# adolliou/euispice_coreg

Hardware: AMD Instinct MI355X
Metric: lag-points/sec (whole node) on 2048² grid, 60×60 CRVAL sweep; argmax-shift match (higher is better)
Workload: dtype f64; 1 GPU; headline: Carrington 'fa' 2048x2048 grid lon(200,300) lat(-20,20), 60x60 CRVAL lags arange(-30,30,1) arcsec, small 2048^2 HRIEUV-like, ref 3072^2 FSI-like, order 2, solar_r 1.004; lag_points=3600, parallelism=single GPU, no collective, resident=True, sweeps_in_flight=2, small_stored_f32=True, use_lds=True

## Files before the change

euispice_coreg_amd/_lib.py:

```python
from __future__ import annotations

import ctypes as C
import os

import numpy as np

_HERE = os.path.dirname(os.path.abspath(__file__))
LIB_PATH = os.environ.get("COREG_HIP_LIB", os.path.join(_HERE, "libcoreg_hip.so"))

COREG_OK = 0
COREG_EINVAL, COREG_EHIP, COREG_ESTATE, COREG_ENOTIMPL, COREG_ENOMEM = -1, -2, -3, -4, -5
COREG_F32, COREG_F64 = 0, 1
PROJ_TAN, PROJ_CAR = 0, 1
METHOD_CORRELATION, METHOD_RESIDUS, METHOD_RESIDUS_MASKED = 0, 1, 2
METHOD_MUTUAL_INFORMATION = 3
CDELT_INTENDED, CDELT_REFERENCE = 0, 1


class CoregError(RuntimeError):
    def __init__(self, code, msg):
        super().__init__(f"libcoreg_hip error {code}: {msg}")
        self.code = code


# ... 211 lines not shown
     [_P, _WP, C.POINTER(CarrGrid), C.c_double, C.POINTER(Lags), C.c_int, C.c_int, C.c_int, C.c_int64, C.c_int64, _P,
      C.c_int]),
    ("coreg_sweep_set_bins", C.c_int, [_P, _P, C.c_int32, _P, C.c_int32]),
    ("coreg_sweep_helioprojective", C.c_int,
     [_P, _WP, _WP, C.POINTER(Lags), C.c_int, C.c_int, C.c_int, C.c_int64, C.c_int64, _P, C.c_int]),
    ("coreg_sums_size", C.c_int, [_P, C.POINTER(C.c_int64)]),
    ("coreg_copy_sums", C.c_int, [_P, _P, C.c_int]),
    ("coreg_finalize_sums", C.c_int, [_P, _P, C.c_int, _P, C.c_int]),
    ("coreg_get_pivots", C.c_int, [_P, C.POINTER(C.c_double)]),
    ("coreg_set_pivots", C.c_int, [_P, C.POINTER(C.c_double)]),
    ("coreg_last_stats", C.c_int, [_P, C.POINTER(Stats)]),
    ("coreg_last_counts", C.c_int, [_P, _P, C.c_int]),
    ("coreg_last_visit_counts", C.c_int, [_P, C.POINTER(C.c_int64)]),
    ("coreg_last_tap_fix", C.c_int, [_P, C.POINTER(C.c_int64)]),
    ("coreg_last_sweep_variant", C.c_int, [_P, C.POINTER(C.c_int32)]),
    ("coreg_set_option", C.c_int, [_P, C.c_char_p, C.c_int64]),
    ("coreg_shift_header", C.c_int,
     [_WP, C.c_double, C.c_double, C.c_double, C.c_double, C.c_double, C.c_int, _WP]),
    ("coreg_homography", C.c_int, [_WP, _WP, C.POINTER(C.c_double)]),
    ("coreg_lag_homography", C.c_int,
     [_WP, _WP, C.POINTER(Lags), C.POINTER(C.c_int32), C.c_int, C.POINTER(C.c_double)]),
    ("coreg_carrington_origin", C.c_int, [_WP, C.POINTER(C.c_double), C.POINTER(C.c_double)]),
    ("coreg_diffrot_table", C.c_int, [C.POINTER(CarrGrid), C.POINTER(DiffRot), _P]),
    ("coreg_car_map", C.c_int, [_WP, _WP, C.c_int64, _P, _P, _P, _P]),
    ("coreg_wcslib_pixel_to_pixel", C.c_int, [_WP, _WP, C.c_int64, _P, _P, _P, _P, _P, _P]),
    ("coreg_car_tile_margin", C.c_int, [_WP, _WP, C.c_int32, C.c_double, C.POINTER(C.c_double)]),
    ("coreg_nansum_planes_be", C.c_int, [_P, C.c_int32, C.c_int64, _P, C.c_int32, _P]),
    ("coreg_fit_gaussian2d", C.c_int,
     [C.c_int32, _P, _P, _P, _P, _P, _P, C.c_int32, C.c_double, C.c_double, C.c_double, C.c_int32, _P,
      C.POINTER(C.c_int32), C.POINTER(C.c_int32)]),
# ... 558 lines not shown
        self._chk(self._lib.coreg_finalize_sums(self._h, _P(sptr), s_dev, _P(int(out_dev_ptr)), 1))
        return None

    def get_pivots(self):
        p = (C.c_double * 2)()
        self._chk(self._lib.coreg_get_pivots(self._h, p))
        return float(p[0]), float(p[1])

    def set_pivots(self, pivot_ref, pivot_small):
        p = (C.c_double * 2)(float(pivot_ref), float(pivot_small))
        self._chk(self._lib.coreg_set_pivots(self._h, p))

    def last_stats(self) -> dict:
        s = Stats()
        self._chk(self._lib.coreg_last_stats(self._h, C.byref(s)))
        return {f: getattr(s, f) for f, _ in Stats._fields_}

    def last_counts(self, dst_ptr=None):
        n = getattr(self, "_counts_n", None)
        if n is None:
            raise CoregError(COREG_ESTATE, "last_counts: no sweep has run through this object")
        if dst_ptr is not None:
            self._chk(self._lib.coreg_last_counts(self._h, _P(int(dst_ptr)), 1))
            return None
        out = np.empty(int(n), dtype=np.float64)
        self._chk(self._lib.coreg_last_counts(self._h, out.ctypes.data, 0))
        return out

    def last_visit_counts(self) -> dict:
        c = (C.c_int64 * 6)()
        self._chk(self._lib.coreg_last_visit_counts(self._h, c))
# ... 360 lines not shown
```

euispice_coreg_amd/csrc/abi_host.hpp:

```cpp
#pragma once
extern "C" {
int coreg_shift_header(const coreg_wcs2d* ref, double d_crval1, double d_crval2, double d_cdelt1, double d_cdelt2,
                       double d_crota, int cdelt_semantics, coreg_wcs2d* out) {
    if (!ref || !out) return COREG_EINVAL;
    return shift_header(*ref, d_crval1, d_crval2, d_cdelt1, d_cdelt2, d_crota, cdelt_semantics, out);
}

int coreg_car_map(const coreg_wcs2d* from, const coreg_wcs2d* to, int64_t n, const double* px, const double* py,
                  double* ox, double* oy) {
    if (!from || !to || n < 0 || (n > 0 && (!px || !py || !ox || !oy))) return COREG_EINVAL;
    if (from->proj != COREG_PROJ_CAR || to->proj != COREG_PROJ_CAR) return COREG_EINVAL;
    CarMapHost m;
    if (m.init(*from, *to)) return 1;
    for (int64_t i = 0; i < n; ++i) m.apply(px[i], py[i], &ox[i], &oy[i]);
    return COREG_OK;
}

int coreg_last_visit_counts(coreg_handle* h, int64_t* counts6) {
    int64_t* counts5 = counts6;
    if (!h || !counts5) return COREG_EINVAL;
    RETCHK(bind_device(h));
    HIPCHK(hipStreamSynchronize(h->stream));
    long long info[8] = {0, 0, 0, 0, 0, 0, 0, 0};
    if (h->tile_info.p) HIPCHK(hipMemcpy(info, h->tile_info.p, 7 * sizeof(long long), hipMemcpyDeviceToHost));
// ... 2 lines not shown
    if (h->counters.p) HIPCHK(hipMemcpy(refined, h->counters.p, sizeof(refined), hipMemcpyDeviceToHost));
    counts5[4] = refined[0];
    counts6[5] = refined[1];
    return COREG_OK;
}

int coreg_last_tap_fix(coreg_handle* h, int64_t* counts3) {
    if (!h || !counts3) return COREG_EINVAL;
    for (int k = 0; k < 3; ++k) counts3[k] = h->tap_last[k];
    return COREG_OK;
}

int coreg_last_sweep_variant(coreg_handle* h, int32_t* v7) {
    if (!h || !v7) return COREG_EINVAL;
    for (int k = 0; k < 7; ++k) v7[k] = h->last_variant[k];
    return COREG_OK;
}

int coreg_car_tile_margin(const coreg_wcs2d* hdr_target, const coreg_wcs2d* hdr_shifted, int32_t tile_w,
                          double tile_abs_lat_rad, double* margin_px) {
    if (!hdr_target || !hdr_shifted || !margin_px || tile_w < 1 || tile_w > kTilePts) return COREG_EINVAL;
    if (hdr_target->proj != COREG_PROJ_CAR || hdr_shifted->proj != COREG_PROJ_CAR) return COREG_EINVAL;
    CarMapHost m;
    if (m.init(*hdr_target, *hdr_shifted)) return 1;
    *margin_px = car_tile_margin(car_box_c(*hdr_target, *hdr_shifted, tile_w), tile_abs_lat_rad + car_pole_sep(m.r));
    return COREG_OK;
}

int coreg_homography(const coreg_wcs2d* from, const coreg_wcs2d* to, double* h9) {
    if (!from || !to || !h9) return COREG_EINVAL;
// ... 118 lines not shown
```

euispice_coreg_amd/csrc/abi_images.hpp:

```cpp
#pragma once
extern "C" {
static int check_image(coreg_handle* h, const void* img, int32_t ny, int32_t nx, const char* who) {
    if (!img || ny < 1 || nx < 1 || too_many(ny, nx))
        return fail(h, COREG_EINVAL, std::string(who) + ": bad image (null pointer, empty, or more than 2^31 - 1 pixels)");
    return COREG_OK;
}
static bool is_dtype(int dtype) { return dtype == COREG_F32 || dtype == COREG_F64; }

static int adopt_small(coreg_handle* h, int32_t ny, int32_t nx, bool f32, hipStream_t s) {
    h->sW = nx;
    h->sH = ny;
    h->small_f32 = f32;
    HIPCHK(buffer_mean(h, h->small.p, f32, (long long)ny * nx, h->pivots.as<double>() + 1, s));
    return end_small_upload(h, s);
}

static int set_small_from(coreg_handle* h, const void* src, const PixFmt& fmt, SrcKind kind, int32_t ny, int32_t nx) {
    RETCHK(check_image(h, src, ny, nx, "set_small"));
    const size_t n = (size_t)ny * nx;
    if (kind == SRC_HOST && (fmt.raw() ? fmt.swap_only() : fmt.f32)) {
        trace("set_small_f32: enter");
        RETCHK(bind_device(h));
        HIPCHK(h->small.reserve(n * sizeof(float)));
        hipStream_t s;
        RETCHK(begin_small_upload(h, &s));
        if (h->opt_async_upload && s != h->stream) {
            h->small_f32 = true;
            h->sW = nx;
            h->sH = ny;
            void* dev = h->small.p;
            const bool swap32 = fmt.raw();
            post_upload(h, [h, dev, src, n, swap32, s] { return upload_small_worker(h, dev, src, n, swap32, s); });
            h->small_pending = true;
            trace("set_small_f32: handed to the upload thread");
            return COREG_OK;
        }
        RETCHK(staged_upload(h, h->small.p, src, n * sizeof(float), s));
        if (fmt.raw()) fits_swap32(h->small.p, n, s);
        RETCHK(adopt_small(h, ny, nx, true, s));
        trace("set_small_f32: issued");
        return COREG_OK;
    }
    RETCHK(bind_device(h));
    bool f32 = true;
// ... 110 lines not shown
        const int64_t len = coregrice::rice_encode_tile(q.data(), npx, blocksize, bytepix, heap + used, heap_cap - used);
        if (len < 0) return COREG_ENOMEM;
        tile_offset[n] = used;
        tile_nbytes[n] = (int32_t)len;
        used += len;
    }
    *heap_used = used;
    return COREG_OK;
}

int coreg_threshold_small(coreg_handle* h, int has_min, double vmin, int has_max, double vmax, long long* n_finite) {
    if (!h) return COREG_EINVAL;
    if (!h->small.p) return fail(h, COREG_ESTATE, "coreg_set_small has not been called");
    RETCHK(bind_device(h));
    const long long n = (long long)h->sW * h->sH;
    if (has_min || has_max) {
        const int nb = (int)std::min<long long>((n + 255) / 256, 2048);
        if (h->small_f32)
            hipLaunchKernelGGL((k_threshold<float>), dim3(nb), dim3(256), 0, h->stream, h->small.as<float>(), n, has_min,
                               vmin, has_max, vmax);
        else
            hipLaunchKernelGGL((k_threshold<double>), dim3(nb), dim3(256), 0, h->stream, h->small.as<double>(), n, has_min,
                               vmin, has_max, vmax);
        HIPCHK(hipGetLastError());
    }
    HIPCHK(buffer_mean(h, h->small.p, h->small_f32, n, h->pivots.as<double>() + 1, h->stream));
    if (n_finite) {
        long long cnt[256];
        HIPCHK(hipMemcpyAsync(cnt, h->red_cnt.p, sizeof(cnt), hipMemcpyDeviceToHost, h->stream));
        HIPCHK(hipStreamSynchronize(h->stream));
// ... 356 lines not shown
```

euispice_coreg_amd/csrc/abi_sweeps.hpp:

```cpp
#pragma once
namespace {

int check_method(coreg_handle* h, int method, bool mi_ok) {
    if (method == COREG_METHOD_MUTUAL_INFORMATION) {
        if (!mi_ok)
            return fail(h, COREG_ENOTIMPL, "method COREG_METHOD_MUTUAL_INFORMATION is a score of coreg_sweep_carrington only: the "
                                           "noise-decided samples of the other header-shift sweeps are corrected as Pearson sums");
        return check_sweep_mi(h);
    }
    if (method != COREG_METHOD_CORRELATION && method != COREG_METHOD_RESIDUS && method != COREG_METHOD_RESIDUS_MASKED)
        return fail(h, COREG_ENOTIMPL,
                    "method must be COREG_METHOD_CORRELATION, COREG_METHOD_RESIDUS or COREG_METHOD_RESIDUS_MASKED");
    return COREG_OK;
}

template <typename OwnChecks>
int open_sweep(coreg_handle* h, ComboRange combo, OwnChecks own_checks, const coreg_lags* lags, int order, int method,
               bool mi_ok, int sem, int64_t lag_begin, int64_t lag_end, int grid_w, int grid_h, const char* grid_what,
               double* corr_out, int out_on_device, SweepCall* call) {
    RETCHK(check_method(h, method, mi_ok));
    RETCHK(check_order(h, order));
    RETCHK(own_checks());
    RETCHK(check_lags(h, lags, &call->d, lag_begin, lag_end, combo));
    RETCHK(bind_device_nowait(h));
// ... 261 lines not shown
}

int coreg_get_pivots(coreg_handle* h, double* pivots2) {
    if (!h || !pivots2) return COREG_EINVAL;
    RETCHK(bind_device(h));
    HIPCHK(hipMemcpyAsync(pivots2, h->pivots.p, 2 * sizeof(double), hipMemcpyDeviceToHost, h->stream));
    HIPCHK(hipStreamSynchronize(h->stream));
    return COREG_OK;
}

int coreg_set_pivots(coreg_handle* h, const double* pivots2) {
    if (!h || !pivots2) return COREG_EINVAL;
    if (!(pivots2[0] == pivots2[0]) || !(pivots2[1] == pivots2[1]) || std::isinf(pivots2[0]) || std::isinf(pivots2[1]))
        return fail(h, COREG_EINVAL, "set_pivots: pivots must be finite");
    RETCHK(bind_device(h));
    HIPCHK(hipMemcpyAsync(h->pivots.p, pivots2, 2 * sizeof(double), hipMemcpyHostToDevice, h->stream));
    HIPCHK(hipStreamSynchronize(h->stream));
    return COREG_OK;
}

int coreg_last_counts(coreg_handle* h, double* dst, int dst_on_device) {
    if (!h) return COREG_EINVAL;
    if (h->counts_n < 0) return fail(h, COREG_ESTATE, "last_counts: no sweep has run on this handle");
    if (!dst && h->counts_n > 0) return fail(h, COREG_EINVAL, "last_counts: dst is null");
    RETCHK(bind_device(h));
    if (h->counts_n > 0)
        HIPCHK(hipMemcpyAsync(dst, h->counts.p, (size_t)h->counts_n * sizeof(double),
                              dst_on_device ? hipMemcpyDeviceToDevice : hipMemcpyDeviceToHost, h->stream));
    HIPCHK(hipStreamSynchronize(h->stream));
    return COREG_OK;
// ... 12 lines not shown
```

euispice_coreg_amd/csrc/coreg_hip.hip:

```cpp
#include <hip/hip_runtime.h>

#include <algorithm>
#include <chrono>
#include <cmath>
#include <cstdio>
#include <cstdlib>
#include <cstring>
#include <limits>
#include <condition_variable>
#include <map>
#include <memory>
#include <mutex>
#include <string>
#include <thread>
#include <functional>
#include <type_traits>
#include <utility>
#include <vector>

#include "fit.hpp"
#include "geometry.hpp"
#include "kernels.hpp"
#include <atomic>
#include "ricecomp.hpp"
// ... 82 lines not shown

int coreg_synchronize(coreg_handle* h) {
    if (!h) return COREG_EINVAL;
    RETCHK(bind_device(h));
    HIPCHK(hipStreamSynchronize(h->stream));
    return COREG_OK;
}

int coreg_set_option(coreg_handle* h, const char* name, int64_t value) {
    if (!h || !name) return COREG_EINVAL;
    const std::string n(name);
    if (n == "use_lds") {
        h->opt_use_lds = value ? 1 : 0;
    } else if (n == "clean_path") {
        h->opt_clean_path = value ? 1 : 0;
    } else if (n == "tap_nan_filter") {
        if (value < 0 || value > 2) return fail(h, COREG_EINVAL, "tap_nan_filter must be 0, 1 or 2");
        h->opt_tap_nan_filter = value;
    } else if (n == "overlap_upload") {
        h->opt_overlap_upload = value ? 1 : 0;
    } else if (n == "async_upload") {
        h->opt_async_upload = value ? 1 : 0;
    } else if (n == "refine") {
        h->opt_refine = value ? 1 : 0;
    } else if (n == "refine_cond_log10") {
        if (value < -3 || value > 15) return fail(h, COREG_EINVAL, "refine_cond_log10 must be in [-3, 15]");
        h->opt_refine_cond_log10 = value;
    } else if (n == "refine_max") {
        if (value < 0 || value > 16) return fail(h, COREG_EINVAL, "refine_max must be in [0, 16]");
    } else if (n == "tile_w") {
// ... 76 lines not shown
```

euispice_coreg_amd/csrc/host_state.hpp:

```cpp
#pragma once
namespace {

enum SrcKind {
    SRC_HOST = 0,
    SRC_PINNED = 1,
    SRC_DEVICE = 2,
    SRC_TILED = 3,
};

struct PixFmt {
    int bitpix = 0;
    bool f32 = false;
    double bscale = 1.0, bzero = 0.0;
    bool raw() const { return bitpix != 0; }
    bool scaled() const { return bscale != 1.0 || bzero != 0.0; }
    size_t elem() const { return raw() ? (size_t)(bitpix < 0 ? -bitpix : bitpix) / 8 : (f32 ? 4 : 8); }
    bool swap_only() const { return bitpix == -32 && !scaled(); }
    static PixFmt native(bool is_f32) {
        PixFmt f;
        f.f32 = is_f32;
        return f;
    }
};

// ... 29 lines not shown
struct ContextState;
struct PixelsState;

struct coreg_handle {
    int device = 0;
    Stream stream;
    std::string err;

    std::unique_ptr<ContextState> ctx;
    std::unique_ptr<PixelsState> pix;
    ~coreg_handle();

    DevBuf small;
    int sW = 0, sH = 0;
    bool small_f32 = false;
    DevBuf ref;
    int gW = 0, gH = 0;
    int ref_dtype = -1;
    DevBuf pivots, red_sum, red_cnt;
    DevBuf t_sin_lon, t_cos_lon, t_cos_lat, t_sin_lat, t_lon_deg, t_dx;
    coreg_diffrot rot_ref = {}, rot_small = {};
    bool has_rot_ref = false, has_rot_small = false;
    CarrTables tabs;
    std::vector<double> tabs_key;
    bool tabs_uploaded = false;
    PinBuf pin_img[2];
    Event ev_img[2];
    int pin_img_next = 0;
    DevBuf pts, tile_count, tile_list, tile_cum, group_first, tile_info, tile_bbox;
    DevBuf visit_rec;
// ... 67 lines not shown
    int64_t opt_crop_reference = 1;
    int64_t opt_taper_min = 128, opt_taper_frac = -1, opt_taper_rounds = 6;
    int64_t opt_use_lds = 1, opt_clean_path = 1, opt_refine = 1, opt_refine_cond_log10 = 5, opt_tile_w = 0, opt_n_groups = 0, opt_lds_bytes = (159 * 1024 * kPointGroups) / 4, opt_patch_w = 0, opt_h_series = 1, opt_h_incr = 1, opt_tile_skip = 1, opt_pitch = -1;

    coreg_stats stats;
    bool stats_pending = false;
    PinBuf pin_info;
    std::vector<EventPair> ev_sweep, ev_pre;
    size_t ev_sweep_used = 0, ev_pre_used = 0;
    hipEvent_t ev_t1 = nullptr;
    Event ev_end[2];
    PinBuf pin_plan[2];
    int plan_slot = 0;
    bool plan_open = false;
};
```

euispice_coreg_amd/csrc/host_sweep_io.hpp:

```cpp
#pragma once
namespace {
int collect_stats(coreg_handle* h);

void reset_stats(coreg_handle* h, long long n_grid_points, long long n_lags) {
    std::memset(&h->stats, 0, sizeof(h->stats));
    h->stats.small_is_f32 = h->small_f32 ? 1 : 0;
    h->stats.n_grid_points = n_grid_points;
    h->stats.n_lags = n_lags;
}

int begin_sweep(coreg_handle* h, long long n_out, double* corr_out, int out_on_device, double** out_dev) {
    h->stats_pending = false;
    h->pending_fin.clear();
    h->sums_slots = 0;
    h->pending_n_out = 0;
    h->tap_last[0] = h->tap_last[1] = h->tap_last[2] = 0;
    h->last_variant[0] = -1;
    std::memset(&h->pending_prologue, 0, sizeof(h->pending_prologue));
    if (h->plan_open) {
        h->plan_open = false;
        RETCHK(bind_device(h));
        HIPCHK(hipStreamSynchronize(h->stream));
    }
    if (!h->small.p) return fail(h, COREG_ESTATE, "coreg_set_small has not been called");
    if (!h->ref.p) return fail(h, COREG_ESTATE, "no reference image on the target grid");
    if (!corr_out && n_out > 0) return fail(h, COREG_EINVAL, "corr_out is null");
    h->ev_sweep_used = 0;
    h->ev_pre_used = 0;
    reset_stats(h, (long long)h->gW * h->gH, n_out);
    if (out_on_device) {
        *out_dev = corr_out;
    } else {
// ... 108 lines not shown
```

euispice_coreg_amd/csrc/host_sweep_launch.hpp:

```cpp
#pragma once
namespace {
using sweep_variant::SweepVariant;
static_assert(sweep_variant::kTranslate == MODE_TRANSLATE && sweep_variant::kHomography == MODE_HOMOGRAPHY &&
                  sweep_variant::kHomographySeries == MODE_HOMOGRAPHY_SERIES && sweep_variant::kCar == MODE_CAR &&
                  sweep_variant::kOrderRt == ORDER_RT, "sweep_variant.hpp restates the kernels' constants");

struct SweepLaunchSpec {
    int mode = MODE_TRANSLATE;
    int order = 2;
    int method = COREG_METHOD_CORRELATION;
    size_t slot_off = 0;
    int n_batches = 0, n_tiles = 0;
    long long lag_begin = 0;
    double* out_dev = nullptr;
    const LaunchU* car_inv = nullptr;
    const BorderFix* fix = nullptr;
    int pitch_sel = 0;
    long long n_slots() const { return (long long)n_batches * kBlock; }
    bool residus() const { return method != COREG_METHOD_CORRELATION; }
    int residus_kind() const { return method == COREG_METHOD_RESIDUS_MASKED ? 2 : (residus() ? 1 : 0); }
    const double* params_dev(const coreg_handle* h) const {
        return h->lane_params.as<double>() + (mode == MODE_TRANSLATE ? 2 : 9) * slot_off;
    }
    const long long* outidx_dev(const coreg_handle* h) const { return h->out_index.as<long long>() + slot_off; }
};

struct SweepKernel {
    void (*fn)(const SweepArgs);
    size_t attr_bytes[kMaxDevices];
};
template <size_t... I>
SweepKernel* sweep_kernel_table(std::index_sequence<I...>) {
    constexpr const SweepVariant* v = sweep_variant::kSweepVariants.v;
    static SweepKernel table[] = {
        {k_sweep<v[I].mode, v[I].order, std::conditional_t<v[I].f32, float, double>, v[I].round, v[I].resid, v[I].pitch>, {0}}...};
    return table;
}

int raise_dynamic_lds(coreg_handle* h, SweepKernel* k, size_t lds_bytes) {
    std::lock_guard<std::mutex> lock(g_attr_mutex);
    size_t& ab = k->attr_bytes[h->device % kMaxDevices];
    if (lds_bytes > 48 * 1024 && lds_bytes > ab) {
        HIPCHK(hipFuncSetAttribute((const void*)k->fn, hipFuncAttributeMaxDynamicSharedMemorySize, (int)lds_bytes));
        ab = lds_bytes;
    }
    return COREG_OK;
}

int sweep_grid(coreg_handle* h, const SweepKernel* k, size_t lds_bytes, long long items, unsigned* grid) {
    long long resident = h->opt_sweep_wgs;
// ... 1 lines not shown
        if (h->n_cus <= 0) HIPCHK(hipDeviceGetAttribute(&h->n_cus, hipDeviceAttributeMultiprocessorCount, h->device));
        int per_cu = 0;
        for (const coreg_handle::SweepResidency& r : h->sweep_residency)
            if (r.fn == (const void*)k->fn && r.lds_bytes == lds_bytes) per_cu = r.per_cu;
        if (per_cu <= 0) {
            HIPCHK(hipOccupancyMaxActiveBlocksPerMultiprocessor(&per_cu, (const void*)k->fn, kSweepThreads, lds_bytes));
            if (per_cu <= 0) return fail(h, COREG_EHIP, "launch_sweep: the device holds no k_sweep workgroup of this LDS size");
            h->sweep_residency.push_back({(const void*)k->fn, lds_bytes, per_cu});
        }
        resident = (long long)h->n_cus * per_cu;
    }
    *grid = (unsigned)(8 * ((std::min(items, resident) + 7) / 8));
    return COREG_OK;
}

int launch_k_sweep(coreg_handle* h, const SweepLaunchSpec& L, SweepArgs a, int n_groups8, size_t lds_bytes) {
    const SweepVariant v = sweep_variant::pick_sweep_variant(L.mode, L.order, h->small_f32, L.residus(), L.pitch_sel);
    const int at = sweep_variant::sweep_variant_index(v);
    if (at < 0) return fail(h, COREG_EINVAL, "launch_sweep: no k_sweep instantiation for this mode / order / pitch");
    SweepKernel* k = sweep_kernel_table(std::make_index_sequence<sweep_variant::kNumSweepVariants>()) + at;
    EventPair* ev = next_event(h, h->ev_sweep, h->ev_sweep_used);
    if (!ev) return fail(h, COREG_EHIP, "hipEventCreate failed");
    RETCHK(raise_dynamic_lds(h, k, lds_bytes));
    a.items8 = n_groups8 * L.n_batches;
    unsigned grid = 0;
    RETCHK(sweep_grid(h, k, lds_bytes, 8LL * a.items8, &grid));
    HIPCHK(h->sweep_queue.reserve(8 * sizeof(unsigned)));
    a.queue = h->sweep_queue.as<unsigned>();
    HIPCHK(hipMemsetAsync(a.queue, 0, 8 * sizeof(unsigned), h->stream));
    HIPCHK(hipEventRecord(ev->a, h->stream));
    hipLaunchKernelGGL(k->fn, dim3(grid), dim3(kSweepThreads), lds_bytes, h->stream, a);
    HIPCHK(hipEventRecord(ev->b, h->stream));
    HIPCHK(hipGetLastError());
    const int rec[7] = {at, v.mode, v.order, v.f32 ? 1 : 0, v.round ? 1 : 0, v.resid ? 1 : 0, v.pitch};
    std::copy(rec, rec + 7, h->last_variant);
// ... 13 lines not shown
    a.tile_info = h->tile_info.as<long long>();
    a.tile_bbox = h->tile_bbox.as<double>();
    a.visit_rec = h->visit_rec.as<VisitRec>();
    a.lane_params = L.params_dev(h);
    a.n_slots = L.n_slots();
    a.n_batches = L.n_batches;
    a.n_groups = n_groups;
    a.group_lo = group_lo;
    a.partials = h->partials.as<double>();
    a.queue = nullptr;
    a.items8 = 0;
    a.pivots = h->pivots.as<double>();
    a.use_lds = h->opt_use_lds ? 1 : 0;
    a.clean_path = h->opt_clean_path ? 1 : 0;
    a.lds_elems = (int)(lds_bytes / sizeof(double));
    a.car_inv = L.car_inv ? *L.car_inv : LaunchU{};
    a.car_inv.order_rt = L.order;
    a.car_inv.h_incr = (int)h->opt_h_incr;
    return a;
}

template <typename Args>
void fill_fix_common(Args& x, const coreg_handle* h, const SweepLaunchSpec& L) {
    x.img = h->small.p;
    x.W = h->sW;
    x.H = h->sH;
    x.ref = h->ref.p;
    x.ref_f32 = h->ref_dtype == COREG_F32 ? 1 : 0;
    x.gw = h->gW;
    x.order = L.order;
    x.round_f32 = L.mode == MODE_TRANSLATE ? 0 : 1;
    x.residus = L.residus() ? 1 : 0;
    x.pivots = h->pivots.as<double>();
    x.hom = L.params_dev(h);
// ... 70 lines not shown
    return COREG_OK;
}

int launch_sweep(coreg_handle* h, const SweepLaunchSpec& L) {
    const long long n_slots = L.n_slots();
    const int n_groups = pick_groups(h, L.n_batches, L.n_tiles);
    const bool sharded = h->opt_shard_world > 1;
    const int g_per = sharded ? n_groups / (int)h->opt_shard_world : n_groups;
    const int g_lo = sharded ? g_per * (int)h->opt_shard_rank : 0;
    const bool fixing = L.fix && L.fix->any() && (!sharded || h->opt_shard_rank == 0);
    HIPCHK(h->partials.reserve((size_t)(g_per + (fixing ? 1 : 0)) * kNumSums * n_slots * sizeof(double)));
    double* fix_slab = fixing ? h->partials.as<double>() + (size_t)g_per * kNumSums * n_slots : nullptr;
    const size_t lds_min = (size_t)(kPointGroups - 1) * kNumSums * kBlock * sizeof(double);
    const size_t lds_bytes = std::max(lds_min, h->opt_use_lds ? (size_t)h->opt_lds_bytes : 0);

    const SweepArgs a = sweep_args(h, L, n_groups, g_lo, lds_bytes);
    RETCHK(join_small(h));
    trace("launch_sweep: launching k_sweep");
    if (g_per % 8 != 0) return fail(h, COREG_EINVAL, "launch_sweep: the groups of a launch must be a multiple of 8");
    RETCHK(launch_k_sweep(h, L, a, g_per / 8, lds_bytes));
    h->stats.n_sweep_launches++;
    h->stats.used_lds = a.use_lds;

    FixLaunch fl;
    RETCHK(build_fix_launch(h, L, &fl));
    if (fixing) {
        HIPCHK(hipMemsetAsync(fix_slab, 0, (size_t)kNumSums * n_slots * sizeof(double), h->stream));
        RETCHK(launch_fix_kernels(h, fl, fix_slab, nullptr, nullptr));
    }

    const bool refinable = h->opt_refine && !L.residus();
    FinalizeArgs f = {};
    RETCHK(fill_refine(h, &f.refine, L.mode, L.order, a.lane_params, a.car_inv, n_slots));
    f.refine.enabled = (refinable && !sharded) ? 1 : 0;
    if (fixing && f.refine.enabled) {
// ... 31 lines not shown
```

euispice_coreg_amd/csrc/kernels_common.hpp:

```cpp
#pragma once
#include "launch_uniforms.hpp"
#include "spline_last.hpp"
namespace coreg {

#ifndef COREG_POINT_GROUPS
#define COREG_POINT_GROUPS 4
#endif
constexpr int kPointGroups = COREG_POINT_GROUPS;
constexpr int kSweepThreads = kBlock * kPointGroups;
constexpr int kChunk = 4;
constexpr int kNumSums = 6;

struct __attribute__((aligned(32))) Pt {
    double b0, b1, a, pad;
};

__host__ __device__ inline double car_tile_margin(double box_c, double th_abs) {
    if (!(th_abs < 1.5)) return __builtin_inf();
    const double c = cos(th_abs);
    return 1.0 + box_c * 2.0 / (c * c);
}

struct CarrDev {
    const double* sin_lon;
// ... 355 lines not shown
```

euispice_coreg_amd/csrc/kernels_prepare.hpp:

```cpp
#pragma once
namespace coreg {
template <typename T>
__global__ void __launch_bounds__(256) k_sum_finite(const T* __restrict__ v, long long n, double* part_sum,
                                                    long long* part_cnt) {
    __shared__ double ss[256];
    __shared__ long long sc[256];
    double s = 0.0;
    long long c = 0;
    for (long long i = (long long)blockIdx.x * 256 + threadIdx.x; i < n; i += (long long)gridDim.x * 256) {
        const double x = (double)v[i];
        if (isfinite(x)) {
            s += x;
            ++c;
        }
    }
    ss[threadIdx.x] = s;
    sc[threadIdx.x] = c;
    __syncthreads();
    for (int o = 128; o > 0; o >>= 1) {
        if ((int)threadIdx.x < o) {
            ss[threadIdx.x] += ss[threadIdx.x + o];
            sc[threadIdx.x] += sc[threadIdx.x + o];
        }
        __syncthreads();
// ... 415 lines not shown
    }
    __syncthreads();
    for (int g = threadIdx.x; g <= n_groups; g += 1024) {
        const long long start = group_start(g, total, n_groups, taper_min, taper_frac);
        group_first[1024 + g] = (int)start;
        int lo = 0, hi = n_list;
        while (lo < hi) {
            const int mid = (lo + hi + 1) >> 1;
            if (mid <= n_list && (long long)tile_cum[mid] <= start) lo = mid;
            else hi = mid - 1;
        }
        group_first[g] = lo;
    }
}

}
```

euispice_coreg_amd/csrc/kernels_sweep.hpp:

```cpp
#pragma once
namespace coreg {
struct SweepArgs {
    const void* img;
    int W, H;
    const Pt* pts;
    const int* tile_count;
    const int* tile_list;
    const int* tile_cum;
    const int* group_first;
    long long* tile_info;
    const double* tile_bbox;
    const VisitRec* visit_rec;
    const double* lane_params;
    long long n_slots;
    int n_batches;
    int n_groups;
    int group_lo;
    double* partials;
    unsigned* queue;
    int items8;
    const double* pivots;
    int use_lds;
    int clean_path;
    int lds_elems;
    LaunchU car_inv;
};

struct Acc {
    int n;
    double a, b, aa, bb, ab;
};

template <int N>
struct Taps;
template <>
struct Taps<3> {
    double t[9];
    __device__ __forceinline__ void issue(unsigned a0, unsigned a1, unsigned a2) {
        asm volatile(
// ... 584 lines not shown
            acc.aa += pt[2].pad;
        }
    }
#endif
    if (pg == n_full % kPointGroups) {
        for (int p = n_full * kChunk; p < p_end; ++p) {
            Pt pt;
            load_pt_uniform(pts + p, pt);
            point_lag<MODE, ORDER, TS, LDS, ROUND, RESID, INTERIOR, PITCH>(acc, win, img, pitch, ox, oy, W, H, wmax, hmax,
                                                                           px0, py0, pxw, pyw, hm, cu, pt.b0, pt.b1, pt.a,
                                                                           pt.pad, pivot_b);
        }
    }
}

template <int MODE, int ORDER, typename TS, bool ROUND, bool RESID, int PITCH = 0>
__global__ void __launch_bounds__(kSweepThreads) k_sweep(const SweepArgs a) {
    extern __shared__ __align__(16) unsigned char lds_raw[];
    double* lds = (double*)lds_raw;
    constexpr int kWaves = kSweepThreads / 64;
    constexpr int kLagWaves = kBlock / 64;
    __shared__ double wred2[2][kLagWaves][4];
    __shared__ int wdirty[2][kWaves];
    constexpr bool kCleanPath = MODE != MODE_CAR && !RESID && ORDER != ORDER_RT && !(ROUND && sizeof(TS) == 8);
    int n_vis = 0, n_vis_lds = 0, n_vis_int = 0, n_vis_clean = 0;

    __shared__ int next_q[2];
    const int slot8 = blockIdx.x & 7;
    int q = blockIdx.x >> 3;
    int item_par = 0;

    const int lane = threadIdx.x & 63, wave = threadIdx.x >> 6;
    const int pg = __builtin_amdgcn_readfirstlane(wave % kPointGroups);
    const int lw = __builtin_amdgcn_readfirstlane(wave / kPointGroups);
    const int ls = 64 * lw + lane;

    const TS* __restrict__ img = (const TS*)a.img;
    const int W = a.W, H = a.H;
    const double inf = __builtin_inf();
    const double pivot_b = a.pivots[1];
#if defined(__HIP_DEVICE_COMPILE__)
    const unsigned win = (unsigned)(uintptr_t)(__attribute__((address_space(3))) unsigned char*)lds_raw;
#else
    const unsigned win = 0;
#endif

    while (q < a.items8) {
    const int batch = q % a.n_batches;
    const int group = a.group_lo + (q / a.n_batches) * 8 + slot8;
    const long long slot = (long long)batch * kBlock + ls;
    int visit = 0;

    double px0 = 0.0, py0 = 0.0;
    H9 hm;
#pragma unroll
// ... 147 lines not shown
          if (in_lds) {
            swept = true;
            ++n_vis_lds;
#ifndef COREG_STAGE_ROWS
#define COREG_STAGE_ROWS 8
#endif
#ifndef COREG_STAGE_COLS
#define COREG_STAGE_COLS 1
#endif
            constexpr int kStage = COREG_STAGE_ROWS, kCols = COREG_STAGE_COLS;
            const double scale = ORDER == 2 ? 0.25 : 1.0;
            constexpr bool kFmaStage = ORDER == 2 && !ROUND && COREG_VISIT_FMA;
            const double npivot4 = -0.25 * pivot_b;
            const int wave_u = __builtin_amdgcn_readfirstlane(wave);
            double poison = 0.0;
            for (int r0 = wave_u; r0 < wh; r0 += kWaves * kStage) {
                for (int c0 = 0; c0 < ww; c0 += 64 * kCols) {
                    int gx[kCols];
#pragma unroll
                    for (int j = 0; j < kCols; ++j) {
                        const int c = c0 + 64 * j + lane;
                        gx[j] = kWide ? mirror_far(ox + min(c, ww - 1), W) : mirror_idx(ox + min(c, ww - 1), W);
                    }
                    TS v[kStage][kCols];
#pragma unroll
                    for (int k = 0; k < kStage; ++k) {
                        const int r = min(r0 + k * kWaves, wh - 1);
                        const int gy = kWide ? mirror_far(oy + r, H) : mirror_idx(oy + r, H);
                        const TS* __restrict__ row = img + (size_t)gy * W;
#pragma unroll
// ... 6 lines not shown
#pragma unroll
                            for (int k = 0; k < kStage; ++k) {
                                const int r = r0 + k * kWaves;
                                if (r < wh) {
                                    const double e = (kFmaStage ? fma((double)v[k][j], 0.25, npivot4)
                                                                : (ROUND ? (double)v[k][j] : (double)v[k][j] - pivot_b) * scale);
                                    lds[r * pitch + c] = e;
                                    if (kCleanPath) poison = fma(e, 0.0, poison);
                                }
                            }
                        }
                    }
                }
            }
            park = park_visit(nxt, park);
            if (kCleanPath && interior) {
                const int dirty = __ballot(poison != poison) != 0ull;
                if (lane == 0) wdirt[wave] = dirty;
            }
            __syncthreads();
            bool done = false;
            if constexpr (ORDER != ORDER_RT) {
                if (interior) {
                    done = true;
                    bool clean = false;
                    if constexpr (kCleanPath) clean = a.clean_path && __ballot(wdirt[lane % kWaves] != 0) == 0ull;
                    ++n_vis_int;
                    n_vis_clean += clean ? 1 : 0;
                    if (!pad_lane) {
                        const double offx = (ORDER == 2 ? 0.5 : 0.0) - (double)(ORDER / 2 + ox);
                        const double offy = (ORDER == 2 ? 0.5 : 0.0) - (double)(ORDER / 2 + oy);
                        const double pxw = MODE == MODE_TRANSLATE ? px0 + offx : offx;
                        const double pyw = MODE == MODE_TRANSLATE ? py0 + offy : offy;
                        if (kCleanPath && clean) {
                            tile_points<MODE, ORDER, TS, true, ROUND, RESID, true, PITCH, kCleanPath>(
                                acc, win, img, pitch, ox, oy, W, H, px0, py0, pxw, pyw, hm, a.car_inv, pts, p_begin, p_end,
                                pivot_b, pg);
                        } else {
                            tile_points<MODE, ORDER, TS, true, ROUND, RESID, true, PITCH>(acc, win, img, pitch, ox, oy, W, H,
                                                                                          px0, py0, pxw, pyw, hm, a.car_inv,
                                                                                          pts, p_begin, p_end, pivot_b, pg);
// ... 67 lines not shown
```

include/coreg_hip.h:

```cpp
#ifndef COREG_HIP_H
#define COREG_HIP_H

#include <stdint.h>

#ifdef __cplusplus
extern "C" {
#endif

#define COREG_OK 0
#define COREG_EINVAL (-1)
#define COREG_EHIP (-2)
#define COREG_ESTATE (-3)
#define COREG_ENOTIMPL (-4)
#define COREG_ENOMEM (-5)

#define COREG_F32 0
#define COREG_F64 1
#define COREG_I32 2

#define COREG_PROJ_TAN 0
#define COREG_PROJ_CAR 1

#define COREG_METHOD_CORRELATION 0
#define COREG_METHOD_RESIDUS 1
// ... 156 lines not shown
int coreg_sums_size(coreg_handle* h, int64_t* n_doubles);
int coreg_copy_sums(coreg_handle* h, double* dst, int dst_on_device);
int coreg_finalize_sums(coreg_handle* h, const double* sums, int sums_on_device, double* corr_out, int out_on_device);

int coreg_get_pivots(coreg_handle* h, double* pivots2);
int coreg_set_pivots(coreg_handle* h, const double* pivots2);

int coreg_last_stats(coreg_handle* h, coreg_stats* out);

int coreg_last_counts(coreg_handle* h, double* dst, int dst_on_device);

int coreg_last_visit_counts(coreg_handle* h, int64_t* counts6);
int coreg_last_tap_fix(coreg_handle* h, int64_t* counts3);

int coreg_last_sweep_variant(coreg_handle* h, int32_t* v7);

int coreg_set_option(coreg_handle* h, const char* name, int64_t value);

int coreg_shift_header(const coreg_wcs2d* ref, double d_crval1, double d_crval2, double d_cdelt1, double d_cdelt2,
                       double d_crota, int cdelt_semantics, coreg_wcs2d* out);
int coreg_homography(const coreg_wcs2d* from, const coreg_wcs2d* to, double* h9);
int coreg_lag_homography(const coreg_wcs2d* hdr_target, const coreg_wcs2d* hdr_small, const coreg_lags* lags,
                         const int32_t idx[5], int cdelt_semantics, double* h9);
int coreg_wcslib_pixel_to_pixel(const coreg_wcs2d* from, const coreg_wcs2d* to, int64_t n, const double* px,
                                const double* py, double* ox, double* oy, double* lng, double* lat);
int coreg_carrington_origin(const coreg_wcs2d* hdr, double* x0, double* y0);
int coreg_diffrot_table(const coreg_carr_grid* grid, const coreg_diffrot* rot, double* dx);
int coreg_car_map(const coreg_wcs2d* from, const coreg_wcs2d* to, int64_t n, const double* px, const double* py,
                  double* ox, double* oy);
int coreg_car_tile_margin(const coreg_wcs2d* hdr_target, const coreg_wcs2d* hdr_shifted, int32_t tile_w,
// ... 108 lines not shown
```

Baseline: 1.268 million lag-points/s.

## Stage sweep LDS windows from a cached pre-scaled padded image with direct DMA

Adds a cached prepared copy of the small image: mirror-padded by one pixel, converted to f64 and pre-scaled as 0.25*v - 0.25*pivot, plus a 2D prefix-sum table of non-finite pixels. The order-2 translate sweep then fills its LDS window from this image, either with plain loads or with global_load_lds direct-to-LDS copies. It checks window cleanliness with four prefix-sum lookups instead of a per-element NaN ballot. The aim is to remove mirror indexing, type conversion, scaling and NaN reduction from every window fill. In exchange it uses an extra f64 buffer and int table, runs a one-time prep when the small image or pivots change, and adds three kernel instantiations per variant.

```diff
diff --git a/euispice_coreg_amd/_lib.py b/euispice_coreg_amd/_lib.py
--- a/euispice_coreg_amd/_lib.py
+++ b/euispice_coreg_amd/_lib.py
@@ -249,6 +249,7 @@
     ("coreg_last_visit_counts", C.c_int, [_P, C.POINTER(C.c_int64)]),
     ("coreg_last_tap_fix", C.c_int, [_P, C.POINTER(C.c_int64)]),
     ("coreg_last_sweep_variant", C.c_int, [_P, C.POINTER(C.c_int32)]),
+    ("coreg_last_sweep_stage", C.c_int, [_P, C.POINTER(C.c_int32)]),
     ("coreg_set_option", C.c_int, [_P, C.c_char_p, C.c_int64]),
     ("coreg_shift_header", C.c_int,
      [_WP, C.c_double, C.c_double, C.c_double, C.c_double, C.c_double, C.c_int, _WP]),
@@ -837,7 +838,11 @@
     def last_stats(self) -> dict:
         s = Stats()
         self._chk(self._lib.coreg_last_stats(self._h, C.byref(s)))
-        return {f: getattr(s, f) for f, _ in Stats._fields_}
+        out = {f: getattr(s, f) for f, _ in Stats._fields_}
+        stage = C.c_int32(0)
+        self._chk(self._lib.coreg_last_sweep_stage(self._h, C.byref(stage)))
+        out["stage"] = stage.value
+        return out
 
     def last_counts(self, dst_ptr=None):
         n = getattr(self, "_counts_n", None)
diff --git a/euispice_coreg_amd/csrc/abi_host.hpp b/euispice_coreg_amd/csrc/abi_host.hpp
--- a/euispice_coreg_amd/csrc/abi_host.hpp
+++ b/euispice_coreg_amd/csrc/abi_host.hpp
@@ -40,6 +40,12 @@
 int coreg_last_sweep_variant(coreg_handle* h, int32_t* v7) {
     if (!h || !v7) return COREG_EINVAL;
     for (int k = 0; k < 7; ++k) v7[k] = h->last_variant[k];
+    return COREG_OK;
+}
+
+int coreg_last_sweep_stage(coreg_handle* h, int32_t* stage) {
+    if (!h || !stage) return COREG_EINVAL;
+    *stage = h->last_stage;
     return COREG_OK;
 }
 
diff --git a/euispice_coreg_amd/csrc/abi_images.hpp b/euispice_coreg_amd/csrc/abi_images.hpp
--- a/euispice_coreg_amd/csrc/abi_images.hpp
+++ b/euispice_coreg_amd/csrc/abi_images.hpp
@@ -11,12 +11,14 @@
     h->sW = nx;
     h->sH = ny;
     h->small_f32 = f32;
+    small_changed(h);
     HIPCHK(buffer_mean(h, h->small.p, f32, (long long)ny * nx, h->pivots.as<double>() + 1, s));
     return end_small_upload(h, s);
 }
 
 static int set_small_from(coreg_handle* h, const void* src, const PixFmt& fmt, SrcKind kind, int32_t ny, int32_t nx) {
     RETCHK(check_image(h, src, ny, nx, "set_small"));
+    small_changed(h);
     const size_t n = (size_t)ny * nx;
     if (kind == SRC_HOST && (fmt.raw() ? fmt.swap_only() : fmt.f32)) {
         trace("set_small_f32: enter");
@@ -28,6 +30,7 @@
             h->small_f32 = true;
             h->sW = nx;
             h->sH = ny;
+            small_changed(h);
             void* dev = h->small.p;
             const bool swap32 = fmt.raw();
             post_upload(h, [h, dev, src, n, swap32, s] { return upload_small_worker(h, dev, src, n, swap32, s); });
@@ -168,6 +171,7 @@
     if (!h->small.p) return fail(h, COREG_ESTATE, "coreg_set_small has not been called");
     RETCHK(bind_device(h));
     const long long n = (long long)h->sW * h->sH;
+    small_changed(h);
     if (has_min || has_max) {
         const int nb = (int)std::min<long long>((n + 255) / 256, 2048);
         if (h->small_f32)
diff --git a/euispice_coreg_amd/csrc/abi_sweeps.hpp b/euispice_coreg_amd/csrc/abi_sweeps.hpp
--- a/euispice_coreg_amd/csrc/abi_sweeps.hpp
+++ b/euispice_coreg_amd/csrc/abi_sweeps.hpp
@@ -299,6 +299,7 @@
     if (!(pivots2[0] == pivots2[0]) || !(pivots2[1] == pivots2[1]) || std::isinf(pivots2[0]) || std::isinf(pivots2[1]))
         return fail(h, COREG_EINVAL, "set_pivots: pivots must be finite");
     RETCHK(bind_device(h));
+    small_changed(h);
     HIPCHK(hipMemcpyAsync(h->pivots.p, pivots2, 2 * sizeof(double), hipMemcpyHostToDevice, h->stream));
     HIPCHK(hipStreamSynchronize(h->stream));
     return COREG_OK;
diff --git a/euispice_coreg_amd/csrc/coreg_hip.hip b/euispice_coreg_amd/csrc/coreg_hip.hip
--- a/euispice_coreg_amd/csrc/coreg_hip.hip
+++ b/euispice_coreg_amd/csrc/coreg_hip.hip
@@ -120,6 +120,9 @@
         h->opt_use_lds = value ? 1 : 0;
     } else if (n == "clean_path") {
         h->opt_clean_path = value ? 1 : 0;
+    } else if (n == "stage") {
+        if (value < 0 || value > 2) return fail(h, COREG_EINVAL, "stage must be 0, 1 or 2");
+        h->opt_stage = value;
     } else if (n == "tap_nan_filter") {
         if (value < 0 || value > 2) return fail(h, COREG_EINVAL, "tap_nan_filter must be 0, 1 or 2");
         h->opt_tap_nan_filter = value;
diff --git a/euispice_coreg_amd/csrc/host_state.hpp b/euispice_coreg_amd/csrc/host_state.hpp
--- a/euispice_coreg_amd/csrc/host_state.hpp
+++ b/euispice_coreg_amd/csrc/host_state.hpp
@@ -67,6 +67,10 @@
     DevBuf small;
     int sW = 0, sH = 0;
     bool small_f32 = false;
+    DevBuf prep, prep_nf;
+    uint64_t small_gen = 1, prep_gen = 0;
+    int64_t opt_stage = 2;
+    int last_stage = 0;
     DevBuf ref;
     int gW = 0, gH = 0;
     int ref_dtype = -1;
@@ -164,3 +168,5 @@
     int plan_slot = 0;
     bool plan_open = false;
 };
+
+static inline void small_changed(coreg_handle* h) { ++h->small_gen; }
diff --git a/euispice_coreg_amd/csrc/host_sweep_io.hpp b/euispice_coreg_amd/csrc/host_sweep_io.hpp
--- a/euispice_coreg_amd/csrc/host_sweep_io.hpp
+++ b/euispice_coreg_amd/csrc/host_sweep_io.hpp
@@ -16,6 +16,7 @@
     h->pending_n_out = 0;
     h->tap_last[0] = h->tap_last[1] = h->tap_last[2] = 0;
     h->last_variant[0] = -1;
+    h->last_stage = 0;
     std::memset(&h->pending_prologue, 0, sizeof(h->pending_prologue));
     if (h->plan_open) {
         h->plan_open = false;
diff --git a/euispice_coreg_amd/csrc/host_sweep_launch.hpp b/euispice_coreg_amd/csrc/host_sweep_launch.hpp
--- a/euispice_coreg_amd/csrc/host_sweep_launch.hpp
+++ b/euispice_coreg_amd/csrc/host_sweep_launch.hpp
@@ -29,11 +29,20 @@
     void (*fn)(const SweepArgs);
     size_t attr_bytes[kMaxDevices];
 };
+constexpr bool stages_from_prepared(const SweepVariant& v) {
+    return v.mode == sweep_variant::kTranslate && v.order == 2 && !v.round;
+}
+constexpr int kSweepStages = 3;
+template <size_t I, int STAGE>
+constexpr auto sweep_kernel_fn() {
+    constexpr SweepVariant v = sweep_variant::kSweepVariants.v[I];
+    return k_sweep<v.mode, v.order, std::conditional_t<v.f32, float, double>, v.round, v.resid, v.pitch,
+                   stages_from_prepared(v) ? STAGE : 0>;
+}
 template <size_t... I>
-SweepKernel* sweep_kernel_table(std::index_sequence<I...>) {
-    constexpr const SweepVariant* v = sweep_variant::kSweepVariants.v;
-    static SweepKernel table[] = {
-        {k_sweep<v[I].mode, v[I].order, std::conditional_t<v[I].f32, float, double>, v[I].round, v[I].resid, v[I].pitch>, {0}}...};
+SweepKernel (*sweep_kernel_table(std::index_sequence<I...>))[kSweepStages] {
+    static SweepKernel table[][kSweepStages] = {
+        {{sweep_kernel_fn<I, 0>(), {0}}, {sweep_kernel_fn<I, 1>(), {0}}, {sweep_kernel_fn<I, 2>(), {0}}}...};
     return table;
 }
 
@@ -65,11 +74,13 @@
     return COREG_OK;
 }
 
-int launch_k_sweep(coreg_handle* h, const SweepLaunchSpec& L, SweepArgs a, int n_groups8, size_t lds_bytes) {
+int launch_k_sweep(coreg_handle* h, const SweepLaunchSpec& L, SweepArgs a, int n_groups8, size_t lds_bytes, int stage) {
     const SweepVariant v = sweep_variant::pick_sweep_variant(L.mode, L.order, h->small_f32, L.residus(), L.pitch_sel);
     const int at = sweep_variant::sweep_variant_index(v);
     if (at < 0) return fail(h, COREG_EINVAL, "launch_sweep: no k_sweep instantiation for this mode / order / pitch");
-    SweepKernel* k = sweep_kernel_table(std::make_index_sequence<sweep_variant::kNumSweepVariants>()) + at;
+    if (stage < 0 || stage >= kSweepStages || (stage != 0 && !(stages_from_prepared(v) && a.prep && a.nf)))
+        return fail(h, COREG_EINVAL, "launch_sweep: this variant does not stage from the prepared image");
+    SweepKernel* k = &sweep_kernel_table(std::make_index_sequence<sweep_variant::kNumSweepVariants>())[at][stage];
     EventPair* ev = next_event(h, h->ev_sweep, h->ev_sweep_used);
     if (!ev) return fail(h, COREG_EHIP, "hipEventCreate failed");
     RETCHK(raise_dynamic_lds(h, k, lds_bytes));
@@ -113,10 +124,49 @@
     a.use_lds = h->opt_use_lds ? 1 : 0;
     a.clean_path = h->opt_clean_path ? 1 : 0;
     a.lds_elems = (int)(lds_bytes / sizeof(double));
+    a.prep = nullptr;
+    a.nf = nullptr;
     a.car_inv = L.car_inv ? *L.car_inv : LaunchU{};
     a.car_inv.order_rt = L.order;
     a.car_inv.h_incr = (int)h->opt_h_incr;
     return a;
+}
+
+int prepared_image(coreg_handle* h) {
+    if (h->prep_gen == h->small_gen && h->prep.p) return COREG_OK;
+    namespace si = stage_image;
+    const int W = h->sW, H = h->sH;
+    HIPCHK(h->prep.reserve((size_t)si::prep_elems(W, H) * sizeof(double)));
+    HIPCHK(h->prep_nf.reserve((size_t)si::nf_elems(W, H) * sizeof(int)));
+    const dim3 grid((unsigned)((si::prep_pitch(W) + 255) / 256), (unsigned)si::prep_rows(H));
+    if (h->small_f32)
+        hipLaunchKernelGGL((k_prep_image<float>), grid, dim3(256), 0, h->stream, h->small.as<float>(), W, H,
+                           h->pivots.as<double>(), h->prep.as<double>());
+    else
+        hipLaunchKernelGGL((k_prep_image<double>), grid, dim3(256), 0, h->stream, h->small.as<double>(), W, H,
+                           h->pivots.as<double>(), h->prep.as<double>());
+    hipLaunchKernelGGL(k_nf_rows, dim3((unsigned)si::nf_rows(H)), dim3(64), 0, h->stream, h->prep.as<double>(), W, H,
+                       h->prep_nf.as<int>());
+    hipLaunchKernelGGL(k_nf_cols, dim3((unsigned)((si::nf_pitch(W) + 255) / 256)), dim3(256), 0, h->stream, W, H,
+                       h->prep_nf.as<int>());
+    HIPCHK(hipGetLastError());
+    h->prep_gen = h->small_gen;
+    return COREG_OK;
+}
+
+int stage_from_prepared(coreg_handle* h, const SweepLaunchSpec& L, SweepArgs* a, int* stage_out) {
+    const SweepVariant v = sweep_variant::pick_sweep_variant(L.mode, L.order, h->small_f32, L.residus(), L.pitch_sel);
+    int stage = (int)h->opt_stage;
+    if (!stages_from_prepared(v) || !a->use_lds || !stage_image::prep_possible(h->sW, h->sH)) stage = 0;
+    if (stage == 2 && !stage_image::dma_fits_launch(v.pitch, a->lds_elems)) stage = 1;
+    if (stage != 0) {
+        RETCHK(prepared_image(h));
+        a->prep = h->prep.as<double>();
+        a->nf = h->prep_nf.as<int>();
+    }
+    *stage_out = stage;
+    h->last_stage = stage;
+    return COREG_OK;
 }
 
 template <typename Args>
@@ -217,11 +267,13 @@
     const size_t lds_min = (size_t)(kPointGroups - 1) * kNumSums * kBlock * sizeof(double);
     const size_t lds_bytes = std::max(lds_min, h->opt_use_lds ? (size_t)h->opt_lds_bytes : 0);
 
-    const SweepArgs a = sweep_args(h, L, n_groups, g_lo, lds_bytes);
+    SweepArgs a = sweep_args(h, L, n_groups, g_lo, lds_bytes);
     RETCHK(join_small(h));
+    int stage = 0;
+    RETCHK(stage_from_prepared(h, L, &a, &stage));
     trace("launch_sweep: launching k_sweep");
     if (g_per % 8 != 0) return fail(h, COREG_EINVAL, "launch_sweep: the groups of a launch must be a multiple of 8");
-    RETCHK(launch_k_sweep(h, L, a, g_per / 8, lds_bytes));
+    RETCHK(launch_k_sweep(h, L, a, g_per / 8, lds_bytes, stage));
     h->stats.n_sweep_launches++;
     h->stats.used_lds = a.use_lds;
 
diff --git a/euispice_coreg_amd/csrc/kernels_common.hpp b/euispice_coreg_amd/csrc/kernels_common.hpp
--- a/euispice_coreg_amd/csrc/kernels_common.hpp
+++ b/euispice_coreg_amd/csrc/kernels_common.hpp
@@ -1,6 +1,7 @@
 #pragma once
 #include "launch_uniforms.hpp"
 #include "spline_last.hpp"
+#include "stage_image.hpp"
 namespace coreg {
 
 #ifndef COREG_POINT_GROUPS
diff --git a/euispice_coreg_amd/csrc/kernels_prepare.hpp b/euispice_coreg_amd/csrc/kernels_prepare.hpp
--- a/euispice_coreg_amd/csrc/kernels_prepare.hpp
+++ b/euispice_coreg_amd/csrc/kernels_prepare.hpp
@@ -453,4 +453,47 @@
     }
 }
 
-}
+template <typename TS>
+__global__ void __launch_bounds__(256) k_prep_image(const TS* __restrict__ img, int W, int H, const double* __restrict__ pivots,
+                                                    double* __restrict__ prep) {
+    const int pp = stage_image::prep_pitch(W);
+    const int cp = blockIdx.x * 256 + threadIdx.x, rp = blockIdx.y;
+    if (cp >= pp) return;
+    const double pivot_b = pivots[1];
+    const double npivot4 = -0.25 * pivot_b;
+    double e = 0.0;
+    if (cp <= W + 1) {
+        const TS v = img[(size_t)stage_image::mirror1(rp - 1, H) * W + stage_image::mirror1(cp - 1, W)];
+        e = fma((double)v, 0.25, npivot4);
+    }
+    prep[(size_t)rp * pp + cp] = e;
+}
+__global__ void __launch_bounds__(64) k_nf_rows(const double* __restrict__ prep, int W, int H, int* __restrict__ nf) {
+    const int pp = stage_image::prep_pitch(W), np = stage_image::nf_pitch(W);
+    const int i = blockIdx.x, lane = threadIdx.x;
+    int* __restrict__ out = nf + (size_t)i * np;
+    if (lane == 0) out[0] = 0;
+    int carry = 0;
+    for (int b = 0; b < W + 2; b += 64) {
+        const int c = b + lane;
+        int x = (i > 0 && c < W + 2 && !isfinite(prep[(size_t)(i - 1) * pp + c])) ? 1 : 0;
+        for (int o = 1; o < 64; o <<= 1) {
+            const int y = __shfl_up(x, o);
+            if (lane >= o) x += y;
+        }
+        if (c < W + 2) out[c + 1] = carry + x;
+        carry += __shfl(x, 63);
+    }
+}
+__global__ void __launch_bounds__(256) k_nf_cols(int W, int H, int* __restrict__ nf) {
+    const int np = stage_image::nf_pitch(W);
+    const int j = blockIdx.x * 256 + threadIdx.x;
+    if (j >= np) return;
+    int acc = 0;
+    for (int i = 1; i < stage_image::nf_rows(H); ++i) {
+        acc += nf[(size_t)i * np + j];
+        nf[(size_t)i * np + j] = acc;
+    }
+}
+
+}
diff --git a/euispice_coreg_amd/csrc/kernels_sweep.hpp b/euispice_coreg_amd/csrc/kernels_sweep.hpp
--- a/euispice_coreg_amd/csrc/kernels_sweep.hpp
+++ b/euispice_coreg_amd/csrc/kernels_sweep.hpp
@@ -23,6 +23,8 @@
     int use_lds;
     int clean_path;
     int lds_elems;
+    const double* prep;
+    const int* nf;
     LaunchU car_inv;
 };
 
@@ -637,7 +639,7 @@
     }
 }
 
-template <int MODE, int ORDER, typename TS, bool ROUND, bool RESID, int PITCH = 0>
+template <int MODE, int ORDER, typename TS, bool ROUND, bool RESID, int PITCH = 0, int STAGE = 0>
 __global__ void __launch_bounds__(kSweepThreads) k_sweep(const SweepArgs a) {
     extern __shared__ __align__(16) unsigned char lds_raw[];
     double* lds = (double*)lds_raw;
@@ -662,6 +664,9 @@
     const int W = a.W, H = a.H;
     const double inf = __builtin_inf();
     const double pivot_b = a.pivots[1];
+    static_assert(STAGE == 0 || (STAGE <= 2 && MODE == MODE_TRANSLATE && ORDER == 2 && !ROUND && COREG_VISIT_FMA),
+                  "only the order-2 translation sweep stages from the prepared image");
+    constexpr bool kFromPrep = STAGE != 0;
 #if defined(__HIP_DEVICE_COMPILE__)
     const unsigned win = (unsigned)(uintptr_t)(__attribute__((address_space(3))) unsigned char*)lds_raw;
 #else
@@ -839,6 +844,47 @@
             const double npivot4 = -0.25 * pivot_b;
             const int wave_u = __builtin_amdgcn_readfirstlane(wave);
             double poison = 0.0;
+            int nf_corner = 0;
+            if constexpr (kFromPrep) {
+                {
+                    if (kCleanPath && interior)
+                        nf_corner = a.nf[(int)stage_image::nf_corner(lane & 3, ox, oy, ex, ey, W)];
+                    const int pp = stage_image::prep_pitch(W);
+                    const double* __restrict__ src0 = a.prep + stage_image::prep_index(oy, ox, W);
+                    if constexpr (STAGE == 2) {
+                        const int half = 4 * lane;
+                        for (int r = wave_u; r < wh; r += kWaves) {
+                            const char* __restrict__ srow = (const char*)(src0 + (size_t)r * pp) + half;
+                            double* lrow = lds + r * pitch;
+                            for (int c0 = 0; c0 < ww; c0 += 32) {
+                                if (c0 + (lane >> 1) < ww)
+                                    __builtin_amdgcn_global_load_lds(
+                                        (const __attribute__((address_space(1))) void*)(srow + 8 * c0),
+                                        (__attribute__((address_space(3))) void*)(lrow + c0), 4, 0, 0);
+                            }
+                        }
+                        asm volatile("s_waitcnt vmcnt(0)" ::: "memory");
+                    } else {
+                        for (int r0 = wave_u; r0 < wh; r0 += kWaves * kStage) {
+                            for (int c0 = 0; c0 < ww; c0 += 64) {
+                                const int c = c0 + lane, gc = min(c, ww - 1);
+                                double v[kStage];
+#pragma unroll
+                                for (int k = 0; k < kStage; ++k)
+                                    v[k] = src0[(size_t)min(r0 + k * kWaves, wh - 1) * pp + gc];
+                                if (c < ww) {
+#pragma unroll
+                                    for (int k = 0; k < kStage; ++k) {
+                                        const int r = r0 + k * kWaves;
+                                        if (r < wh) lds[r * pitch + c] = v[k];
+                                    }
+                                }
+                            }
+                        }
+                    }
+                }
+            }
+            if constexpr (!kFromPrep)
             for (int r0 = wave_u; r0 < wh; r0 += kWaves * kStage) {
                 for (int c0 = 0; c0 < ww; c0 += 64 * kCols) {
                     int gx[kCols];
@@ -875,7 +921,7 @@
                 }
             }
             park = park_visit(nxt, park);
-            if (kCleanPath && interior) {
+            if (kCleanPath && interior && !kFromPrep) {
                 const int dirty = __ballot(poison != poison) != 0ull;
                 if (lane == 0) wdirt[wave] = dirty;
             }
@@ -885,7 +931,13 @@
                 if (interior) {
                     done = true;
                     bool clean = false;
-                    if constexpr (kCleanPath) clean = a.clean_path && __ballot(wdirt[lane % kWaves] != 0) == 0ull;
+                    if constexpr (kCleanPath) {
+                        if constexpr (kFromPrep)
+                            clean = a.clean_path && __builtin_amdgcn_readlane(nf_corner, 0) - __builtin_amdgcn_readlane(nf_corner, 1) -
+                                                            __builtin_amdgcn_readlane(nf_corner, 2) +
+                                                            __builtin_amdgcn_readlane(nf_corner, 3) == 0;
+                        else clean = a.clean_path && __ballot(wdirt[lane % kWaves] != 0) == 0ull;
+                    }
                     ++n_vis_int;
                     n_vis_clean += clean ? 1 : 0;
                     if (!pad_lane) {
diff --git a/euispice_coreg_amd/csrc/stage_image.hpp b/euispice_coreg_amd/csrc/stage_image.hpp
--- /dev/null
+++ b/euispice_coreg_amd/csrc/stage_image.hpp
@@ -0,0 +1,57 @@
+#pragma once
+#if defined(__HIPCC__)
+#define COREG_STAGE_HD __host__ __device__
+#else
+#define COREG_STAGE_HD
+#endif
+namespace coreg {
+namespace stage_image {
+
+COREG_STAGE_HD constexpr int mirror1(int i, int n) {
+    i = i < 0 ? -i : i;
+    i = i > n - 1 ? 2 * (n - 1) - i : i;
+    return i < 0 ? 0 : (i > n - 1 ? n - 1 : i);
+}
+
+COREG_STAGE_HD constexpr int prep_pitch(int W) { return (W + 3) & ~1; }
+COREG_STAGE_HD constexpr int prep_rows(int H) { return H + 2; }
+COREG_STAGE_HD constexpr long long prep_elems(int W, int H) { return (long long)prep_rows(H) * prep_pitch(W); }
+COREG_STAGE_HD constexpr long long prep_index(int r, int c, int W) { return (long long)(r + 1) * prep_pitch(W) + (c + 1); }
+
+COREG_STAGE_HD constexpr int nf_pitch(int W) { return W + 3; }
+COREG_STAGE_HD constexpr int nf_rows(int H) { return H + 3; }
+COREG_STAGE_HD constexpr long long nf_elems(int W, int H) { return (long long)nf_rows(H) * nf_pitch(W); }
+COREG_STAGE_HD constexpr bool prep_possible(int W, int H) {
+    return W >= 1 && H >= 1 && (long long)(H + 3) * (W + 4) < (1LL << 31);
+}
+COREG_STAGE_HD constexpr long long nf_corner(int k, int ox, int oy, int ex, int ey, int W) {
+    return (long long)((k & 2) ? ey + 2 : oy + 1) * nf_pitch(W) + ((k & 1) ? ex + 2 : ox + 1);
+}
+COREG_STAGE_HD constexpr int nf_corner_sign(int k) { return (k == 0 || k == 3) ? 1 : -1; }
+COREG_STAGE_HD inline int nonfinite_in_box(const int* nf, int ox, int oy, int ex, int ey, int W) {
+    int n = 0;
+    for (int k = 0; k < 4; ++k) n += nf_corner_sign(k) * nf[nf_corner(k, ox, oy, ex, ey, W)];
+    return n;
+}
+
+COREG_STAGE_HD constexpr int dma_pieces(int ww) { return (ww + 31) / 32; }
+COREG_STAGE_HD constexpr bool dma_lane_on(int piece, int lane, int ww) { return 32 * piece + (lane >> 1) < ww; }
+COREG_STAGE_HD constexpr long long dma_lane_byte(int r, int piece, int lane, int pitch) {
+    return 8LL * ((long long)r * pitch + 32 * piece) + 4 * lane;
+}
+COREG_STAGE_HD constexpr long long dma_last_byte(int ww, int wh, int pitch) {
+    return 8LL * ((long long)(wh - 1) * pitch + ww) - 1;
+}
+COREG_STAGE_HD constexpr bool window_admitted(int ww, int wh, int pitch, long long lds_elems) {
+    return ww >= 1 && wh >= 1 && ww <= pitch && (long long)pitch * wh <= lds_elems;
+}
+COREG_STAGE_HD constexpr bool dma_fits_launch(int pitch, long long lds_elems) {
+    if (lds_elems < 1 || lds_elems * 8 > (1LL << 30)) return false;
+    const long long p = pitch > 0 ? pitch : lds_elems;
+    const long long wh = lds_elems / p;
+    if (wh < 1) return true;
+    return dma_last_byte((int)p, (int)wh, (int)p) < 8 * lds_elems;
+}
+
+}
+}
diff --git a/include/coreg_hip.h b/include/coreg_hip.h
--- a/include/coreg_hip.h
+++ b/include/coreg_hip.h
@@ -194,6 +194,8 @@
 int coreg_last_tap_fix(coreg_handle* h, int64_t* counts3);
 
 int coreg_last_sweep_variant(coreg_handle* h, int32_t* v7);
+
+int coreg_last_sweep_stage(coreg_handle* h, int32_t* stage);
 
 int coreg_set_option(coreg_handle* h, const char* name, int64_t value);
 
```

New measurement: 1.278 million lag-points/s, median of 6. No clear change (+0.8%).
